# devmentality/LEAStereo

Measured on AMD Instinct MI355X. Metric: stereo pairs/s at 576×960 D=192, 1/2/4/8 GPU; EPE vs reference, higher is better.
Workload: dtype f32; 1 GPU; SceneFlow 576x960 D=192 fp32, batch 1 per GPU (BASELINE configs[1]); height=576, width=960, maxdisp=192, global_batch=1, parallelism=dp1 (pairs sharded over ranks, no collective in the step), launch=hip graph replay

## Files before the change

### include/leastereo_hip.h

```cpp
#ifndef LEASTEREO_HIP_H
#define LEASTEREO_HIP_H

#include <stddef.h>
#include <stdint.h>

#ifdef __cplusplus
extern "C" {
#endif

#define LEA_ABI_VERSION 14

#define LEA_F32 0
#define LEA_BF16 1

#define LEA_OK 0
#define LEA_E_INVALID 1001
#define LEA_E_UNSUPPORTED 1002

#define LEA_RELU 1u
#define LEA_RESIDUAL 2u
#define LEA_PAIR_SUM 4u

int lea_abi_version(void);
const char* lea_last_error(void);
// ... 10 lines not shown
                      const void* x2, int64_t x2_bstride, int cin2,
                      const float* w_packed, const float* scale, const float* shift,
                      const void* residual, int64_t r_bstride,
                      void* y, int64_t y_bstride,
                      int B, int cin, int cout, int D, int H, int W, int k,
                      unsigned flags, int dtype, void* stream);

int lea_conv1x1_heads(const void* x, int64_t x_bstride, const void* x2, int64_t x2_bstride,
                      int cin2, const float* w_packed,
                      const float* scale_a, const float* shift_a, void* y_a, int64_t ya_bstride,
                      int cout_a, unsigned flags_a,
                      const float* scale_b, const float* shift_b, void* y_b, int64_t yb_bstride,
                      int cout_b, unsigned flags_b,
                      int B, int cin, int D, int H, int W, int dtype, void* stream);
const char* lea_conv1x1_heads_kernel_name(int B, int cout, int D, int H, int W);

int lea_conv3d_bnrelu_resampled(const void* x, int64_t x_bstride, int Di, int Hi, int Wi,
                                const float* w_packed, const float* scale, const float* shift,
                                const void* residual, int64_t r_bstride,
                                void* y, int64_t y_bstride,
                                int B, int cin, int cout, int D, int H, int W, int k,
                                unsigned flags, int dtype, void* stream);

int lea_conv3d_bnrelu_costvolume(const void* left, const void* right, int64_t f_bstride,
                                 const float* w_packed, const float* scale, const float* shift,
                                 void* y, int64_t y_bstride, int B, int C, int cout, int D3,
                                 int H, int W, unsigned flags, int dtype, void* stream);
const char* lea_conv3d_costvolume_kernel_name(int B, int cout, int D3, int H, int W);

const char* lea_conv3d_kernel_name(int B, int cout, int D, int H, int W, int k, int resampled);
// ... 291 lines not shown
```

### include/leastereo_hip_tuning.h

```cpp
#ifndef LEASTEREO_HIP_TUNING_H
#define LEASTEREO_HIP_TUNING_H

#ifdef __cplusplus
extern "C" {
#endif

int lea_conv3d_set_tile_override(int nt, int tw, int td);

int lea_conv3d_set_rs_gather(int on);

int lea_conv1x1_set_vector(int on);

int lea_conv3d_bf16_set_tile_override(int th, int td, int mt);

int lea_conv3d_bf16_set_variant(int variant);

int lea_conv3d_bf16_set_stream1x1(int on);

int lea_conv3d_bf16_set_pair_split(int on);

int lea_resample_bf16_set_batch(int k);

int lea_resample_bf16_set_cols(int on);

// ... 25 lines not shown

int lea_conv3d_wino2_set_pipeline(int on);

int lea_conv3d_wino2p_set_wpre(int on);

int lea_conv3d_wino44_set(int on);

int lea_conv3d_wino44_set_upre(int on);

int lea_conv3d_wino44_set_sched(int s);

int lea_conv3d_wino44_set_group(int g);

int lea_conv3d_wino_set_epi_buf(int on);

int lea_conv3d_wino_set_small_cout(int mode);

int lea_conv3d_wino_set_block48(int on);

int lea_rectify_set_tile(int mode);

#ifdef __cplusplus
}
#endif
#endif
```

### leastereo_amd/_lib.py

```python
from __future__ import annotations

import ctypes
import os
import threading

LIB_PATH = os.environ.get(
    "LEASTEREO_HIP_LIB",
    os.path.join(os.path.dirname(os.path.abspath(__file__)), "libleastereo_hip.so"))

ABI_VERSION = 14
LEA_F32 = 0
LEA_BF16 = 1
LEA_RELU = 1
LEA_RESIDUAL = 2
LEA_PAIR_SUM = 4
LEA_CVS_TMAJOR = 8
LEA_E_INVALID = 1001

_p = ctypes.c_void_p
_i = ctypes.c_int
_i64 = ctypes.c_int64
_u = ctypes.c_uint

SIGNATURES = {
    "lea_abi_version": (_i, []),
    "lea_last_error": (ctypes.c_char_p, []),
    "lea_build_cost_volume": (_i, [_p, _p, _p, _i, _i, _i, _i, _i, _i, _p]),
    "lea_conv3d_packed_floats": (ctypes.c_size_t, [_i, _i, _i]),
    "lea_conv3d_pack_weights": (_i, [_p, _p, _i, _i, _i, _p]),
    "lea_conv3d_bnrelu": (_i, [_p, _i64, _p, _i64, _i, _p, _p, _p, _p, _i64, _p, _i64,
                               _i, _i, _i, _i, _i, _i, _i, _u, _i, _p]),
    "lea_conv1x1_heads": (_i, [_p, _i64, _p, _i64, _i, _p, _p, _p, _p, _i64, _i, _u, _p, _p, _p, _i64, _i, _u,
                               _i, _i, _i, _i, _i, _i, _p]),
    "lea_conv1x1_heads_kernel_name": (ctypes.c_char_p, [_i, _i, _i, _i, _i]),
    "lea_conv3d_bnrelu_resampled": (_i, [_p, _i64, _i, _i, _i, _p, _p, _p, _p, _i64, _p, _i64,
                                         _i, _i, _i, _i, _i, _i, _i, _u, _i, _p]),
    "lea_conv3d_kernel_name": (ctypes.c_char_p, [_i, _i, _i, _i, _i, _i, _i]),
    "lea_conv3d_set_tile_override": (_i, [_i, _i, _i]),
    "lea_conv3d_bnrelu_costvolume": (_i, [_p, _p, _i64, _p, _p, _p, _p, _i64, _i, _i, _i, _i, _i,
                                          _i, _u, _i, _p]),
    "lea_conv3d_costvolume_kernel_name": (ctypes.c_char_p, [_i, _i, _i, _i, _i]),
    "lea_conv2d_packed_floats": (ctypes.c_size_t, [_i, _i]),
    "lea_conv2d_pack_weights": (_i, [_p, _p, _i, _i, _p]),
    "lea_conv2d_bnrelu": (_i, [_p, _i64, _p, _p, _p, _p, _i64, _p, _i64, _i, _i, _i, _i, _i, _u,
                               _i, _p]),
    "lea_conv2d_kernel_name": (ctypes.c_char_p, [_i, _i, _i, _i]),
    "lea_conv2d_s3_bnrelu": (_i, [_p, _i64, _p, _p, _p, _p, _i64, _i, _i, _i, _i, _i, _u, _i, _p]),
    "lea_feature_stem_bnrelu": (_i, [_p, _i64, _p, _p, _p, _p, _p, _p, _p, _i64, _i, _i, _i, _i, _i, _i,
                                     _i, _p]),
# ... 83 lines not shown
    "lea_conv3d_wino2_set_halo16": (_i, [_i]),
    "lea_conv3d_wino2_set_lane_halo16": (_i, [_i]),
    "lea_conv3d_wino_set_fence": (_i, [_i]),
    "lea_resample_set_mode": (_i, [_i]),
    "lea_conv2d_set_small": (_i, [_i]),
    "lea_conv2d_kernel_name_cin": (ctypes.c_char_p, [_i, _i, _i, _i, _i]),
    "lea_conv2d_bnrelu_pair": (_i, [_p, _i64, _p, _p, _p, _p, _i64, _p, _i64, _p, _i64, _i, _i, _i, _i, _i,
                                    _i, _u, _p]),
    "lea_conv3d_wino2_set_pipeline": (_i, [_i]),
    "lea_conv3d_wino2p_set_wpre": (_i, [_i]),
    "lea_conv3d_wino44_set": (_i, [_i]),
    "lea_conv3d_wino44_set_upre": (_i, [_i]),
    "lea_conv3d_wino44_set_sched": (_i, [_i]),
    "lea_conv3d_wino44_set_group": (_i, [_i]),
    "lea_conv3d_wino_set_epi_buf": (_i, [_i]),
    "lea_conv3d_set_rs_gather": (_i, [_i]),
    "lea_conv1x1_set_vector": (_i, [_i]),
    "lea_conv3d_bf16_set_stream1x1": (_i, [_i]),
    "lea_conv3d_wino_set_small_cout": (_i, [_i]),
    "lea_conv3d_wino_set_block48": (_i, [_i]),
    "lea_cv_stem_split_weights": (_i, [_p, _p, _p, _i, _i, _p]),
    "lea_cv_stem_combine": (_i, [_p, _i64, _p, _i64, _p, _p, _p, _i64, _i, _i, _i, _i, _i, _u, _i,
                                 _p]),
    "lea_cv_stem_map_windows": (_i, [_i, _i, ctypes.POINTER(_i), ctypes.POINTER(_i)]),
    "lea_conv2d_windowed_tiles": (_i, [_i, _i, _i, _i, _i, ctypes.POINTER(_i)]),
    "lea_conv2d_bnrelu_windowed": (_i, [_p, _i64, _p, _p, _p, _p, _i64, _i, _i, _i, _i, _i, _i, _i, _i, _i, _i,
                                        _u, _i, _p]),
    "lea_cv_stem_down2_supported": (_i, [_i, _i, _i, _i, _i]),
    "lea_cv_stem_combine_down2": (_i, [_p, _i64, _p, _i64, _p, _p, _p, _i64, _p, _i64, _i, _i, _i, _i, _i,
                                       _u, _i, _p]),
# ... 54 lines not shown
            _lib = lib
    return _lib


TUNING_ENV = {"LEASTEREO_WINO2_WALK": "lea_conv3d_wino2_set_walk",
              "LEASTEREO_HALO16": "lea_conv3d_wino2_set_halo16",
              "LEASTEREO_LANE_HALO16": "lea_conv3d_wino2_set_lane_halo16",
              "LEASTEREO_WINO_FENCE": "lea_conv3d_wino_set_fence",
              "LEASTEREO_RESAMPLE_MODE": "lea_resample_set_mode",
              "LEASTEREO_CONV2D_SMALL": "lea_conv2d_set_small",
              "LEASTEREO_WINO2_PIPE": "lea_conv3d_wino2_set_pipeline",
              "LEASTEREO_WINO2P_WPRE": "lea_conv3d_wino2p_set_wpre",
              "LEASTEREO_WINO44": "lea_conv3d_wino44_set",
              "LEASTEREO_WINO44_UPRE": "lea_conv3d_wino44_set_upre",
              "LEASTEREO_EPI_BUF": "lea_conv3d_wino_set_epi_buf",
              "LEASTEREO_RS_GATHER": "lea_conv3d_set_rs_gather",
              "LEASTEREO_1X1_VEC": "lea_conv1x1_set_vector",
              "LEASTEREO_BF16_1X1": "lea_conv3d_bf16_set_stream1x1",
              "LEASTEREO_RESAMPLE_K": "lea_resample_bf16_set_batch",
              "LEASTEREO_RESAMPLE_COLS": "lea_resample_bf16_set_cols",
              "LEASTEREO_W22": "lea_conv3d_wino_set_w22",
              "LEASTEREO_PAIR_SPLIT": "lea_conv3d_bf16_set_pair_split",
              "LEASTEREO_DISP_REG": "lea_disparity_set_register_form",
              "LEASTEREO_TAPSUM_ROWS": "lea_tapsum_set_rows"}


def _apply_env_tuning(lib):
    for var, fn in TUNING_ENV.items():
        if os.environ.get(var):
            if getattr(lib, fn)(int(os.environ[var])) != 0:
# ... 8 lines not shown
```

### leastereo_amd/csrc/conv3d.hip

```cpp
#include "conv3d_impl.h"

namespace lea {

template <int KS, int MT, int NT, int TW, bool RS>
__global__ __launch_bounds__(kConvThreads, 2) void conv3d_reg_kernel(const ConvArgs a) {
  using C = TileCfg<KS, MT, NT, TW>;
  constexpr int CIN_B = C::CIN_B;
  __shared__ __attribute__((aligned(16))) float smem[C::STAGE];
  __shared__ Axis tabs[RS ? (KS + C::RH + C::RW) : 1];
  float* xs = smem;
  float* ws = smem + C::XS;

  const int tid = threadIdx.x;
  const int lane = tid & 63;
  const int wave = tid >> 6;
  const int tile = blockIdx.x;
  const int h0 = (tile / a.tiles_w) * C::TH;
  const int w0 = (tile % a.tiles_w) * TW;
  const int d0 = blockIdx.y;
  const int b = blockIdx.z / a.ncob;
  const int co0 = (blockIdx.z - b * a.ncob) * C::COP;
  const int nchunks = (a.cin + CIN_B - 1) / CIN_B;
  const float* wp = a.wp + (long long)(co0 / C::COP) * nchunks * C::WS;
  const long long HW = (long long)a.H * a.W;
// ... 297 lines not shown
      }
    }
  }
}

template <int MT, int NT, bool VEC>
__global__ __launch_bounds__(kConvThreads) void conv1x1_kernel(const ConvArgs a) {
  conv1x1_body<MT, NT, VEC, false>(a, Conv1x1HeadB{});
}

template <int MT, int NT, bool VEC>
__global__ __launch_bounds__(kConvThreads) void conv1x1_heads_kernel(const ConvArgs a, const Conv1x1HeadB hb) {
  conv1x1_body<MT, NT, VEC, true>(a, hb);
}

template <int COUT>
__global__ __launch_bounds__(kConvThreads) void conv3d_valu_kernel(const ConvArgs a) {
  constexpr int TH = 8, TW = 64, RH = TH + 2, RW = TW + 2, PLANE = RH * RW, IMG = 3 * PLANE;
  constexpr int CIN_B = PackCfg<3, 1>::CIN_B;
  constexpr int CIS = (IMG + 15) / 16 * 16;
  constexpr int STAGE = CIN_B * CIS;
  constexpr int XSLOTS = (IMG + 63) / 64;
  constexpr int XSLOTS_W = (XSLOTS + kConvWaves - 1) / kConvWaves;
  constexpr int CHUNK = PackCfg<3, 1>::CHUNK;
  __shared__ __attribute__((aligned(16))) float smem[2 * STAGE];

  const int tid = threadIdx.x;
  const int lane = tid & 63;
  const int wave = __builtin_amdgcn_readfirstlane(tid >> 6);
  const int h0 = (blockIdx.x / a.tiles_w) * TH;
// ... 564 lines not shown
  a.wp = w_packed;
  a.scale = scale_a;
  a.shift = shift_a;
  a.y = (float*)y_a;
  a.ybs = ya_bstride;
  a.cin = cin;
  a.cout = cout_a + cout_b;
  a.D = D;
  a.H = H;
  a.W = W;
  a.flags = flags_a;
  const Conv1x1HeadB hb{(float*)y_b, yb_bstride, scale_b, shift_b, cout_a, flags_b};
  const Plan p = make_plan(B, a.cout, D, H, W, 1, false);
  a.ncob = (a.cout + p.mt * 16 - 1) / (p.mt * 16);
  return run_1x1(p, a, B, as_stream(stream), &hb);
}

extern "C" size_t lea_conv2d_packed_floats(int cout, int cin) {
  if (cout <= 0 || cin <= 0) return 0;
  return lea::packed_floats_2d(cout, cin);
}

extern "C" int lea_conv2d_pack_weights(const float* w, float* packed, int cout, int cin,
                                       void* stream) {
  using namespace lea;
  clear_error();
  LEA_CHECK_ARG(w && packed, "lea_conv2d_pack_weights: null pointer");
  LEA_CHECK_ARG(cout > 0 && cin > 0, "lea_conv2d_pack_weights: bad shape cout=%d cin=%d", cout, cin);
  const long long total = (long long)packed_floats_2d(cout, cin);
  const int threads = 256;
// ... 252 lines not shown
```

### leastereo_amd/csrc/conv3d_wino.hip

```cpp
#include "wino_common.h"

namespace lea {
namespace wino {

template <int F, int Q, int MT, int NP, int TD, bool H16 = false>
struct Cfg {
  static constexpr bool DP = MT == 0;
  static constexpr int MTE = DP ? 1 : MT;
  static constexpr int TDA = DP ? 1 : TD;
  static constexpr int NSTEP = DP ? 12 : 9;
  static_assert(!DP || TD == 2, "a depth-paired tile covers two output planes");
  static constexpr int NX = F + 2;
  static constexpr int COP = 16 * MTE;
  static constexpr bool SWZ = (COP % 32) == 0;
  static constexpr int RPG = 16 / Q;
  static constexpr int TW = F * Q;
  static constexpr int TH = 4 * NP * RPG;
  static constexpr int RH = TH + 2, RW = TW + 2;
  static constexpr int PLANE = RH * RW;
  static constexpr int PLANES = TD + 2;
  static constexpr int IMG = PLANES * PLANE;
  static constexpr int XSLOTS = (IMG + 63) / 64;
  static constexpr int CIS = conflict_free_cis<F, Q>(64 * XSLOTS, RW);
  static constexpr int RWA = TW + 8;
// ... 53 lines not shown
  const int q8 = nblk / 8, r8 = nblk % 8;
  const int lin = (xcd < r8 ? xcd * (q8 + 1) : r8 * (q8 + 1) + (xcd - r8) * q8) + idx;
  const int spw = a.spw > 0 ? a.spw : 1;
  const int ngz = (a.ndz + spw - 1) / spw;
  const int cob = lin % a.ncob;
  const int rest = lin / a.ncob;
  const int gz = rest % ngz;
  const int tile = (rest / ngz) % a.ntiles;
  const int b = rest / (ngz * a.ntiles);
  const int h0 = (tile / a.tiles_w) * C::TH;
  const int w0 = (tile % a.tiles_w) * C::TW;
  const int dz0 = gz * spw, ngroups = min(spw, a.ndz - dz0);
  const int co0 = cob * C::COP;
  const int nchunks = a.cin / CIN_B;
  const int nitems = ngroups * nchunks;
  const float* wp = a.wp + (long long)cob * nchunks * C::WS;
  const int HW = a.H * a.W;
  const unsigned nrec = (unsigned)(HW * a.D) * 4u;

  unsigned hwo[XSLOTS_W];
  int pln[XSLOTS_W], wco[CV ? XSLOTS_W : 1];
#pragma unroll
  for (int t = 0; t < XSLOTS_W; ++t) {
    const int e = (wave + kConvWaves * t) * 64 + lane;
    unsigned v = 0xFFFFFFF0u;
    int pl = -1000, wc_ = 0;
    if (e < C::IMG) {
      const int p = e / C::PLANE;
      const int r = e - p * C::PLANE;
      const int rr = r / C::RW;
// ... 44 lines not shown
      if constexpr (CV) {
        const bool okc = ok && wco[t] >= d;
        voff[t] = okc ? hwo[t] : 0xFFFFFFF0u;
        voffr[t] = okc ? hwo[t] - (unsigned)d * 4u : 0xFFFFFFF0u;
      } else {
        voff[t] = ok ? hwo[t] + (unsigned)d * (unsigned)HW * 4u : 0xFFFFFFF0u;
      }
    }
  };

  auto issue = [&](int item, float* st) {
    const int ch = item % nchunks;
    if (ch == 0) set_group((dz0 + item / nchunks) * TD);
    const float* wsrc = wp + (long long)ch * C::WS;
    float* wdst = st + C::XS;
#pragma unroll
    for (int t = 0; t < WSLOTS_W; ++t) {
      const int j = wave + kConvWaves * t;
      if (j < WSLOTS)
        dma_dwordx4(wsrc + j * 256 + lane * 4, lds0 + 4 * (unsigned)(wdst - smem + j * 256));
    }
    const long long cvol = CV ? (long long)HW : (long long)HW * a.D;
    const unsigned crec = CV ? (unsigned)HW * 4u : nrec;
    if constexpr (H16) {
#pragma unroll
      for (int t = 0; t < T16; ++t) {
        const int k = wave + kConvWaves * t, ci = k / P16;
        const int c = ch * CIN_B + ci;
        const float* base = c < a.cin1 ? a.x + (long long)b * a.xbs + (long long)c * cvol
                                       : a.x2 + (long long)b * a.x2bs + (long long)(c - a.cin1) * cvol;
        const __amdgpu_buffer_rsrc_t rs = __builtin_amdgcn_make_buffer_rsrc((void*)base, 0, crec, 0x00020000);
        const int cb = C::cbh(0) + ci * C::CSH;
        if (ok16[t]) dma_dwordx4_buf(rs, voff16[t], lds0 + 4 * (unsigned)(st - smem + cb + (k % P16) * 256));
      }
      return;
// ... 468 lines not shown
}

struct Plan {
  int f, q, mt, np, td;
  bool d2;
  Plan2 p2;
  bool h16;
};

int g_override[3] = {0, 0, 0};
int g_variant = 0;
int g_spw = 0;
int g_small16 = 0;
int g_block48 = 1;
int g_epibuf = 1;
int g_halo16 = 1;
int g_pipe = 1;
int g_wpre = 1;
int g_fence = 1;
int g_lane16 = 2;
int g_w22 = 0;
inline int host_mt(int cout) {
  if (g_small16 && cout <= 8) return 1;
  const int mt = mt_of(cout);
  return (mt == 3 && !g_block48) ? 2 : mt;
}
inline long long staged_floats(int cout, int cin) {
  const int mt = host_mt(cout), cop = cop_of(mt), nstep = mt == 0 ? 12 : 9;
  return (long long)((cout + cop - 1) / cop) * (cin / CIN_B) * nstep * 3 * CIN_B * cop + 256;
}
// ... 111 lines not shown
    conv3d_wino_kernel<F, Q, MT, NP, TD, CV><<<dim3((unsigned)n_), kConvThreads, 0, st>>>(a); \
    return launch_status("lea_conv3d(wino)");                                                \
  }
#define LEA_WINO_TILES(CV)                                                                                  \
  LEA_WINO_CASE(2, 16, 1, 1, 1, CV) LEA_WINO_CASE(2, 16, 1, 1, 2, CV) LEA_WINO_CASE(2, 16, 1, 2, 1, CV)     \
  LEA_WINO_CASE(2, 16, 1, 2, 2, CV) LEA_WINO_CASE(2, 16, 2, 1, 1, CV) LEA_WINO_CASE(2, 16, 2, 1, 2, CV)     \
  LEA_WINO_CASE(2, 16, 2, 2, 1, CV) LEA_WINO_CASE(2, 16, 2, 2, 2, CV) LEA_WINO_CASE(2, 16, 3, 1, 1, CV)     \
  LEA_WINO_CASE(2, 16, 3, 1, 2, CV) LEA_WINO_CASE(4, 16, 1, 1, 1, CV) LEA_WINO_CASE(4, 16, 1, 1, 2, CV)     \
  LEA_WINO_CASE(4, 16, 2, 1, 1, CV) LEA_WINO_CASE(4, 16, 2, 1, 2, CV) LEA_WINO_CASE(4, 8, 1, 1, 1, CV)      \
  LEA_WINO_CASE(4, 8, 1, 1, 2, CV) LEA_WINO_CASE(4, 8, 2, 1, 1, CV) LEA_WINO_CASE(4, 8, 2, 1, 2, CV)      \
  LEA_WINO_CASE(4, 8, 3, 1, 1, CV) LEA_WINO_CASE(4, 16, 0, 1, 2, CV) LEA_WINO_CASE(4, 8, 0, 1, 2, CV)

int run(const Plan& p, ConvArgs a, int B, hipStream_t st, bool cv) {
  if (p.d2) return run2(p.p2, a, B, st, cv);
  a.ncob = (a.cout + cop_of(p.mt) - 1) / cop_of(p.mt);
  if (p.h16) {
    using C_ = Cfg<4, 16, 0, 1, 2, true>;
    a.tiles_w = (a.W + C_::TW - 1) / C_::TW;
    a.ntiles = a.tiles_w * ((a.H + C_::TH - 1) / C_::TH);
    a.ndz = (a.D + 1) / 2;
    a.spw = std::max(1, std::min(g_spw > 0 ? g_spw : auto_walk(a, B, 2), a.ndz));
    const long long n_ = (long long)a.ntiles * ((a.ndz + a.spw - 1) / a.spw) * B * a.ncob;
    LEA_CHECK_ARG(n_ < (1LL << 31), "lea_conv3d(wino): grid too large");
    a.nblk = (int)n_;
    if (g_fence)
      conv3d_wino_kernel<4, 16, 0, 1, 2, false, true, true><<<dim3((unsigned)n_), kConvThreads, 0, st>>>(a);
    else
      conv3d_wino_kernel<4, 16, 0, 1, 2, false, true><<<dim3((unsigned)n_), kConvThreads, 0, st>>>(a);
    return launch_status("lea_conv3d(wino)");
  }
// ... 129 lines not shown
  wino::g_override[2] = f;
  return 0;
}

extern "C" int lea_conv3d_wino_set_block48(int on) {
  clear_error();
  LEA_CHECK_ARG(on == 0 || on == 1, "lea_conv3d_wino_set_block48: on=%d", on);
  wino::g_block48 = on;
  return 0;
}

extern "C" int lea_conv3d_wino_set_epi_buf(int on) {
  clear_error();
  LEA_CHECK_ARG(on == 0 || on == 1, "lea_conv3d_wino_set_epi_buf: on=%d", on);
  wino::g_epibuf = on;
  return 0;
}

extern "C" int lea_conv3d_wino_set_small_cout(int mode) {
  clear_error();
  LEA_CHECK_ARG(mode == 0 || mode == 1, "lea_conv3d_wino_set_small_cout: mode=%d", mode);
  wino::g_small16 = mode;
  return 0;
}

extern "C" int lea_conv3d_wino2_set_pipeline(int on) {
  clear_error();
  LEA_CHECK_ARG(on == 0 || on == 1, "lea_conv3d_wino2_set_pipeline: on=%d", on);
  wino::g_pipe = on;
  return 0;
// ... 144 lines not shown
  if (B <= 0 || cin <= 0 || cout <= 0 || cout > 8 || D < 2 || H < 2 || W < 4 || D % 2 || H % 2 || W % 4 ||
      cin % CIN_B)
    return 0;
  if ((long long)D * H * W * 4 >= (1LL << 32) || (long long)(cout + 47) * D * H * W >= (1LL << 31)) return 0;
  if (!g_epibuf || g_w22 == 2 || g_variant != 0 || g_override[0] != 0) return 0;
  Plan p = make_plan(B, cout, D, H, W);
  if (p.mt != 0 || p.d2 || p.f != 4 || p.np != 1 || p.td != 2) return 0;
  plan_halo16(p, false, W, a, cin);
  if (a && !epi_buf_ok(*a)) return 0;
  if (p.q == 16) return (p.h16 && g_fence) ? 16 : 0;
  return p.q == 8 ? 8 : 0;
}

static int run_dp_down2(ConvArgs a, int B, int q, bool only, hipStream_t st) {
  a.ncob = 1;
  const int tw = 4 * q, th = 4 * (16 / q);
  a.tiles_w = (a.W + tw - 1) / tw;
  a.ntiles = a.tiles_w * ((a.H + th - 1) / th);
  a.ndz = (a.D + 1) / 2;
  a.spw = std::max(1, std::min(g_spw > 0 ? g_spw : auto_walk(a, B, 2), a.ndz));
  const long long n_ = (long long)a.ntiles * ((a.ndz + a.spw - 1) / a.spw) * B * a.ncob;
  LEA_CHECK_ARG(n_ < (1LL << 31), "lea_conv3d_bnrelu_wino_dp_down2: grid too large");
  a.nblk = (int)n_;
  const dim3 grid((unsigned)n_);
  if (q == 16) {
    if (only)
      conv3d_wino_dp_down2_kernel<16, true><<<grid, kConvThreads, 0, st>>>(a);
    else
      conv3d_wino_dp_down2_kernel<16, false><<<grid, kConvThreads, 0, st>>>(a);
  } else {
// ... 202 lines not shown
```

### leastereo_amd/csrc/wino_common.h

```cpp
#pragma once
#include "conv3d_impl.h"

namespace lea {
namespace wino {

constexpr int CIN_B = 4;

__host__ __device__ constexpr int mt_of(int cout) {
  return cout <= 8 ? 0 : cout <= 16 ? 1 : (cout % 32 != 0 && cout % 48 == 0) ? 3 : 2;
}
__host__ __device__ constexpr int cop_of(int mt) { return 16 * (mt > 0 ? mt : 1); }

template <int F, int Q>
__host__ __device__ constexpr int lane_dword(int lane, int cis, int rw) {
  return (lane >> 4) * cis + ((lane & 15) / Q) * rw + F * ((lane & 15) % Q);
}
template <int F, int Q>
__host__ __device__ constexpr int conflict_free_cis(int img, int rw) {
  for (int cis = img + (img & 1);; cis += 2) {
    bool used[64] = {};
    bool ok = true;
    for (int l = 0; l < 32 && ok; ++l)
      for (int k = 0; k < 2 && ok; ++k) {
        const int bank = (lane_dword<F, Q>(l, cis, rw) + k) % 64;
// ... 14 lines not shown
}
__device__ __forceinline__ void dma_dwordx4_buf(__amdgpu_buffer_rsrc_t rs, unsigned voff, unsigned lds) {
  unsigned keep;
  asm volatile("s_mov_b32 %0, m0\n\ts_mov_b32 m0, %3\n\ts_nop 0\n\tbuffer_load_dwordx4 %1, %2, 0 offen lds\n\ts_mov_b32 m0, %0"
               : "=&s"(keep) : "v"(voff), "s"(rs), "s"(lds) : "memory");
}
__device__ __forceinline__ void dma_dwordx4(const float* src, unsigned lds) {
  unsigned keep;
  asm volatile("s_mov_b32 %0, m0\n\ts_mov_b32 m0, %2\n\ts_nop 0\n\tglobal_load_lds_dwordx4 %1, off\n\ts_mov_b32 m0, %0"
               : "=&s"(keep) : "v"(src), "s"(lds) : "memory");
}

__device__ __forceinline__ int a_col(int m, int ci, int n, bool swz) { return ((swz ? (m ^ (ci & 1)) : m) * 16) + n; }

constexpr unsigned kEpiBuf = 1u << 16;
constexpr unsigned kPairSum = LEA_PAIR_SUM;
constexpr unsigned kEpiOob = 0xFFFFFF00u;
typedef unsigned u32x4_t __attribute__((ext_vector_type(4)));
typedef unsigned u32x2_t __attribute__((ext_vector_type(2)));
typedef float f32x2 __attribute__((ext_vector_type(2)));
__device__ __forceinline__ __amdgpu_buffer_rsrc_t block_rsrc(const float* base, long long bytes) {
  return __builtin_amdgcn_make_buffer_rsrc((void*)base, 0, (int)(unsigned)bytes, 0x00020000);
}
__device__ __forceinline__ f32x4 buf_load4(__amdgpu_buffer_rsrc_t rs, unsigned off) {
  return __builtin_bit_cast(f32x4, __builtin_amdgcn_raw_buffer_load_b128(rs, off, 0, 0));
}
__device__ __forceinline__ void buf_store4(__amdgpu_buffer_rsrc_t rs, unsigned off, f32x4 v) {
  __builtin_amdgcn_raw_buffer_store_b128(__builtin_bit_cast(u32x4_t, v), rs, off, 0, 0);
}
template <int NST>
// ... 59 lines not shown
```

### leastereo_amd/executor.py

```python
from __future__ import annotations

import os
from dataclasses import dataclass

import torch

from . import kernels
from .arch import scale_dimension


def _stacked(fl: torch.Tensor, fr: torch.Tensor) -> torch.Tensor:
    if (fl.is_contiguous() and fr.is_contiguous() and fl.shape == fr.shape and fl.dtype == fr.dtype
            and fl.device == fr.device
            and fl.untyped_storage().data_ptr() == fr.untyped_storage().data_ptr()
            and fr.data_ptr() == fl.data_ptr() + fl.numel() * fl.element_size()):
        return fl.as_strided((2 * fl.shape[0],) + tuple(fl.shape[1:]), fl.stride())
    return torch.cat((fl, fr), 0)


@dataclass
class ConvParams:
    packed: torch.Tensor
    scale: torch.Tensor | None
    shift: torch.Tensor | None
# ... 385 lines not shown
                    dst.add_(t)
                else:
                    dst.copy_(t)
                written.add(step)
            states.append(dst)
        return prev_input, out


class MatchingExecutor(CellGraphExecutor):
    SPLIT_S1_GROUP48 = os.environ.get("LEASTEREO_SPLIT_GROUP48", "1") != "0"
    PAIR_STEPS = WINOGRAD and os.environ.get("LEASTEREO_PAIR_STEPS", "0") != "0"
    FUSED_DOWN = os.environ.get("LEASTEREO_FUSED_DOWN", "1") != "0"
    FUSED_DOWN_CELLS = os.environ.get("LEASTEREO_FUSED_DOWN_CELLS", "1") != "0"
    WINDOWED_MAPS = os.environ.get("LEASTEREO_WINDOWED_MAPS", "1") != "0"
    FANOUT_1X1 = os.environ.get("LEASTEREO_FANOUT_1X1", "1") != "0"

    def run(self, x):
        return self._from_stem0(self.conv("stem0", x))

    def run_features(self, fl, fr, maxdisp):
        p = self.p["stem0"]
        if fl.shape[1] * 2 != p.cin:
            raise ValueError(f"stem0 expects {p.cin} cost-volume channels, got 2*{fl.shape[1]}")
        d3 = int(maxdisp / 3)
        if self.cv is not None and kernels.cv_stem_supported(p.cout, d3, fl.shape[3], False):
            return self._from_stem0(*self._cv_stem(fl.unsqueeze(2), fr.unsqueeze(2), d3))
        if p.wino is not None and kernels.wino_preferred(fl.shape[0], p.cout, p.cin, int(maxdisp / 3),
                                                         *fl.shape[2:4]):
            stem0 = kernels.conv3d_bnrelu_costvolume_wino(fl, fr, maxdisp, p.wino, p.cout, p.scale,
                                                          p.shift, p.relu)
# ... 105 lines not shown
                    prev = (outs[4][0], fused)
            elif i == 9 and n == 12:
                fused = self.conv("conv2", outs[4][1], x2=outs[8][1])
                self._emit("conv2", fused)
                prev = (outs[8][0], fused)
            o = self.cell(i, prev[0], prev[1], down=down)
            cell_down, self._cell_down = self._cell_down, None
            self._emit(f"cell{i}", o[1])
            outs.append(o)
            prev = o
        last = outs[-1][1]
        lh = self._volume(last)[1]
        full, half, quarter = (d, h, w), (d // 2, h // 2, w // 2), (d // 4, h // 4, w // 4)
        if lh == h:
            return self._last3_same_size(last)
        if lh == h // 2:
            y = self.conv("last_6", last)
        elif lh == h // 4:
            y = self.conv("last_6", self.conv("last_12", last), size=half)
        elif lh == h // 8:
            y = self.conv("last_12", self.conv("last_24", last), size=quarter)
            y = self.conv("last_6", y, size=half)
        else:
            raise ValueError(f"matching-net output size {tuple(last.shape[2:])} has no head")
        p3 = self.p["last_3"]
        q = self.conv("last_3.taps", y)
        return self._tapsum(q, p3, full)

    @staticmethod
    def _tapsum(q, p3, full):
        return kernels.tapsum_upsample(q, p3.cout, full, p3.scale, p3.shift, p3.relu)

    def _last3_same_size(self, last):
        return self.conv("last_3", last)

    def __init__(self, matching):
        super().__init__(matching)
        with torch.no_grad():
            last3 = matching.last_3.conv.weight
            co, ci = last3.shape[:2]
            taps = last3.permute(0, 2, 3, 4, 1).reshape(co * 27, ci, 1, 1, 1)
            self.p["last_3.taps"] = ConvParams(kernels.pack_conv_weight(taps), None, None,
# ... 3 lines not shown
                wl, wr = kernels.cv_stem_split_weights(matching.stem0.conv.weight)
                self.cv = self._cv_stem_pack(wl, wr)
                if self.WINDOWED_MAPS and not isinstance(self, _C8Layout):
                    co = wl.shape[0] // 9
                    wlt = wl.view(3, 3, co, *wl.shape[1:]).transpose(0, 1).reshape(wl.shape)
                    self.cv_win = (kernels.pack_conv2d_weight_windowed(wlt, 3 * co),
                                   kernels.pack_conv2d_weight_windowed(wr, 3 * co))
        self._use_winograd()


class MatchingExecutorDirect(MatchingExecutor):

    SPLIT_S1_GROUP48 = False
    PAIR_STEPS = False
    FANOUT_1X1 = False

    def __init__(self, matching):
        super().__init__(matching)
        self.cv = self.cv_win = None

    def _use_winograd(self):
        """Direct engine only."""


class FeatureExecutor(CellGraphExecutor):
    FUSED_STEM = os.environ.get("LEASTEREO_FEATURE_STEM", "1") != "0"
    PAIR_S0 = os.environ.get("LEASTEREO_PAIR_S0", "1") != "0"

    def _stems(self, x, c8=False, x2=None):
        p0, p1 = self.p["stem0"], self.p["stem1"]
# ... 89 lines not shown
                                                      p.relu, out)
            x = self._downsampled(x, size)
        if p.kind == "bf16_2d":
            if x2 is not None:
                raise ValueError(f"{name}: 2D conv takes one input")
            return kernels.conv2d_bnrelu_bf16(x, p.packed, p.cout, p.scale, p.shift, p.relu, out,
                                              accumulate, residual)
        return kernels.conv3d_bnrelu_bf16(x, p.packed, p.cout, p.k, p.scale, p.shift, p.relu, out,
                                          accumulate, x2, residual)


class MatchingExecutorBF16(_C8Layout, MatchingExecutor):

    SPLIT_S1_GROUP48 = False
    FANOUT_1X1 = False
    PAIR_STEPS = os.environ.get("LEASTEREO_PAIR_STEPS", "1") != "0"

    def __init__(self, matching):
        from .model import ConvBR
        super().__init__(matching)
        with torch.no_grad():
            for name, p in list(self.p.items()):
                if name == "last_3":
                    continue
                if name == "last_3.taps":
                    w = matching.last_3.conv.weight
                    co, ci = w.shape[:2]
                    taps = w.permute(0, 2, 3, 4, 1).reshape(co * 27, ci, 1, 1, 1)
                    pad = (-taps.shape[0]) % 8
                    taps = torch.cat([taps, taps.new_zeros((pad,) + tuple(taps.shape[1:]))], 0)
# ... 144 lines not shown
```

### leastereo_amd/kernels.py

```python
from __future__ import annotations

import collections
import contextlib
import ctypes
import math
import os

import numpy as np
import torch

from . import _lib
from ._lib import LEA_BF16, LEA_CVS_TMAJOR, LEA_F32, LEA_PAIR_SUM, LEA_RELU, LEA_RESIDUAL, check


def _stream():
    return torch.cuda.current_stream().cuda_stream


ProbeRecord = collections.namedtuple("ProbeRecord", "name flops bytes start end mfma_flops shape")


class KernelProbe:

    def __init__(self, names=None):
# ... 289 lines not shown
        raise ValueError("conv1x1_heads: neither head accumulates or takes a residual")
    _require_cuda(x, x2, packed, scale_a, shift_a, scale_b, shift_b, out_a, out_b)
    b, cin, d, h, w = x.shape
    xbs = _check_volume_view(x, "x")
    x2ptr, x2bs, cin2 = _second_source(x2, b, (d, h, w))
    out_a, abs_ = _out_view(out_a, _act_shape(b, cout_a, (d, h, w)), x.device, name="out_a")
    out_b, bbs = _out_view(out_b, _act_shape(b, cout_b, (d, h, w)), x.device, name="out_b")
    cout = cout_a + cout_b
    _launch("lea_conv1x1_heads", x.data_ptr(), xbs, x2ptr, x2bs, cin2, packed.data_ptr(),
            _ptr(scale_a), _ptr(shift_a), out_a.data_ptr(), abs_, cout_a, _flags(relu_a),
            _ptr(scale_b), _ptr(shift_b), out_b.data_ptr(), bbs, cout_b, _flags(relu_b),
            b, cin + cin2, d, h, w, LEA_F32,
            probe=lambda: _conv_record(b, cin + cin2, cout, d, h, w, 1, False, b * d * h * w, False,
                                       name=_decode(_lib.load().lea_conv1x1_heads_kernel_name(b, cout, d, h, w))))
    return out_a, out_b


def costvolume_kernel_name(b, cout, d3, h, w):
    return _decode(_lib.load().lea_conv3d_costvolume_kernel_name(b, cout, d3, h, w))


def conv3d_bnrelu_costvolume(fl: torch.Tensor, fr: torch.Tensor, maxdisp: int, packed: torch.Tensor,
                             cout: int, scale: torch.Tensor | None, shift: torch.Tensor | None,
                             relu: bool = True) -> torch.Tensor:
    _require_cuda(fl, fr, packed, scale, shift)
    b, c, h, w = _feature_pair(fl, fr)
    d3 = int(maxdisp / 3)
    out = torch.empty((b, cout, d3, h, w), device=fl.device, dtype=fl.dtype)
    _launch("lea_conv3d_bnrelu_costvolume", fl.data_ptr(), fr.data_ptr(), fl.stride(0), packed.data_ptr(),
            _ptr(scale), _ptr(shift), out.data_ptr(), out.stride(0), b, c, cout, d3, h, w, _flags(relu), LEA_F32,
# ... 1337 lines not shown
```

Before: 166.3 pairs/s.

## Fuse head 1x1 conv chain into one kernel and keep Winograd weights resident

```diff
diff --git a/include/leastereo_hip.h b/include/leastereo_hip.h
--- a/include/leastereo_hip.h
+++ b/include/leastereo_hip.h
@@ -48,6 +48,13 @@
                       int cout_b, unsigned flags_b,
                       int B, int cin, int D, int H, int W, int dtype, void* stream);
 const char* lea_conv1x1_heads_kernel_name(int B, int cout, int D, int H, int W);
+
+int lea_conv1x1_chain(const void* x, int64_t x_bstride,
+                      const float* w1_packed, const float* scale1, const float* shift1, unsigned flags1,
+                      const float* w2_packed, const float* scale2, const float* shift2, unsigned flags2,
+                      void* y, int64_t y_bstride,
+                      int B, int c0, int c1, int c2, int D, int H, int W, int dtype, void* stream);
+const char* lea_conv1x1_chain_kernel_name(int B, int c1, int c2, int D, int H, int W);
 
 int lea_conv3d_bnrelu_resampled(const void* x, int64_t x_bstride, int Di, int Hi, int Wi,
                                 const float* w_packed, const float* scale, const float* shift,
diff --git a/include/leastereo_hip_tuning.h b/include/leastereo_hip_tuning.h
--- a/include/leastereo_hip_tuning.h
+++ b/include/leastereo_hip_tuning.h
@@ -63,6 +63,8 @@
 
 int lea_conv3d_wino_set_epi_buf(int on);
 
+int lea_conv3d_wino_set_wresident(int on);
+
 int lea_conv3d_wino_set_small_cout(int mode);
 
 int lea_conv3d_wino_set_block48(int on);
diff --git a/leastereo_amd/_lib.py b/leastereo_amd/_lib.py
--- a/leastereo_amd/_lib.py
+++ b/leastereo_amd/_lib.py
@@ -16,6 +16,7 @@
 LEA_PAIR_SUM = 4
 LEA_CVS_TMAJOR = 8
 LEA_E_INVALID = 1001
+LEA_E_UNSUPPORTED = 1002
 
 _p = ctypes.c_void_p
 _i = ctypes.c_int
@@ -33,6 +34,9 @@
     "lea_conv1x1_heads": (_i, [_p, _i64, _p, _i64, _i, _p, _p, _p, _p, _i64, _i, _u, _p, _p, _p, _i64, _i, _u,
                                _i, _i, _i, _i, _i, _i, _p]),
     "lea_conv1x1_heads_kernel_name": (ctypes.c_char_p, [_i, _i, _i, _i, _i]),
+    "lea_conv1x1_chain": (_i, [_p, _i64, _p, _p, _p, _u, _p, _p, _p, _u, _p, _i64, _i, _i, _i, _i, _i, _i, _i,
+                               _i, _p]),
+    "lea_conv1x1_chain_kernel_name": (ctypes.c_char_p, [_i, _i, _i, _i, _i, _i]),
     "lea_conv3d_bnrelu_resampled": (_i, [_p, _i64, _i, _i, _i, _p, _p, _p, _p, _i64, _p, _i64,
                                          _i, _i, _i, _i, _i, _i, _i, _u, _i, _p]),
     "lea_conv3d_kernel_name": (ctypes.c_char_p, [_i, _i, _i, _i, _i, _i, _i]),
@@ -146,6 +150,7 @@
     "lea_conv3d_wino44_set_sched": (_i, [_i]),
     "lea_conv3d_wino44_set_group": (_i, [_i]),
     "lea_conv3d_wino_set_epi_buf": (_i, [_i]),
+    "lea_conv3d_wino_set_wresident": (_i, [_i]),
     "lea_conv3d_set_rs_gather": (_i, [_i]),
     "lea_conv1x1_set_vector": (_i, [_i]),
     "lea_conv3d_bf16_set_stream1x1": (_i, [_i]),
@@ -230,6 +235,7 @@
               "LEASTEREO_WINO44": "lea_conv3d_wino44_set",
               "LEASTEREO_WINO44_UPRE": "lea_conv3d_wino44_set_upre",
               "LEASTEREO_EPI_BUF": "lea_conv3d_wino_set_epi_buf",
+              "LEASTEREO_WINO_WRES": "lea_conv3d_wino_set_wresident",
               "LEASTEREO_RS_GATHER": "lea_conv3d_set_rs_gather",
               "LEASTEREO_1X1_VEC": "lea_conv1x1_set_vector",
               "LEASTEREO_BF16_1X1": "lea_conv3d_bf16_set_stream1x1",
diff --git a/leastereo_amd/csrc/conv3d.hip b/leastereo_amd/csrc/conv3d.hip
--- a/leastereo_amd/csrc/conv3d.hip
+++ b/leastereo_amd/csrc/conv3d.hip
@@ -335,6 +335,173 @@
   conv1x1_body<MT, NT, VEC, true>(a, hb);
 }
 
+struct Conv1x1Second {
+  const float* wp;
+  const float* scale;
+  const float* shift;
+  int cout;
+  unsigned flags;
+};
+
+constexpr int kChainTile = 32 * 16 + 8 * 16;
+
+__device__ __forceinline__ void wave_lds_sync() {
+  __builtin_amdgcn_fence(__ATOMIC_RELEASE, "wavefront");
+  __builtin_amdgcn_wave_barrier();
+  __builtin_amdgcn_fence(__ATOMIC_ACQUIRE, "wavefront");
+}
+
+template <int MT1, int MT2, int NT, bool VEC>
+__global__ __launch_bounds__(kConvThreads, 5) void conv1x1_chain_kernel(const ConvArgs a, const Conv1x1Second sb) {
+  using P = PackCfg<1, MT1>;
+  using P2 = PackCfg<1, MT2>;
+  static_assert(MT1 <= 2 && MT2 <= 2, "the middle tensor is one cout block and one K chunk");
+  constexpr int CIN_B = P::CIN_B;
+  constexpr int KS = CIN_B / 4;
+  using vecf = float __attribute__((ext_vector_type(NT)));
+  __shared__ __attribute__((aligned(16))) float ws[P::CHUNK];
+  __shared__ __attribute__((aligned(16))) float ws2[P2::CHUNK];
+  __shared__ float tiles[kConvWaves][kChainTile];
+  __shared__ float ep1[2][32];
+  const int tid = threadIdx.x;
+  const int lane = tid & 63;
+  const int wave = tid >> 6;
+  const int b = blockIdx.y;
+  const int nchunks = (a.cin + CIN_B - 1) / CIN_B;
+  const long long V = (long long)a.D * a.H * a.W;
+  const long long v0 = ((long long)blockIdx.x * kConvWaves + wave) * NT * 16;
+  const int kq = lane >> 4, n = lane & 15;
+  auto vox = [&](int j) -> long long { return VEC ? v0 + NT * n + j : v0 + j * 16 + n; };
+  const bool full = VEC && vox(NT - 1) < V;
+
+  {
+    const float4* src = reinterpret_cast<const float4*>(sb.wp);
+    float4* dst = reinterpret_cast<float4*>(ws2);
+#pragma unroll
+    for (int i = tid; i < P2::CHUNK / 4; i += kConvThreads) dst[i] = src[i];
+    if (tid < 32) {
+      ep1[0][tid] = (a.scale && tid < a.cout) ? a.scale[tid] : 1.f;
+      ep1[1][tid] = (a.shift && tid < a.cout) ? a.shift[tid] : 0.f;
+    }
+  }
+
+  constexpr int MTX = MT1 > MT2 ? MT1 : MT2;
+  f32x4 acc[MTX][NT];
+#pragma unroll
+  for (int m = 0; m < MT1; ++m)
+#pragma unroll
+    for (int j = 0; j < NT; ++j) acc[m][j] = f32x4{0.f, 0.f, 0.f, 0.f};
+
+  for (int ch = 0; ch < nchunks; ++ch) {
+    float bv[KS][NT];
+#pragma unroll
+    for (int s = 0; s < KS; ++s) {
+      const int c = ch * CIN_B + 4 * s + kq;
+      const float* src = a.x + (long long)b * a.xbs + (long long)c * V;
+      if (VEC && full && c < a.cin) {
+        const vecf t = *reinterpret_cast<const vecf*>(src + vox(0));
+#pragma unroll
+        for (int j = 0; j < NT; ++j) bv[s][j] = t[j];
+      } else {
+#pragma unroll
+        for (int j = 0; j < NT; ++j) {
+          const long long v = vox(j);
+          bv[s][j] = (c < a.cin && v < V) ? src[v] : 0.f;
+        }
+      }
+    }
+    __syncthreads();
+    {
+      const float4* src = reinterpret_cast<const float4*>(a.wp + (long long)ch * P::CHUNK);
+      float4* dst = reinterpret_cast<float4*>(ws);
+#pragma unroll
+      for (int i = tid; i < P::CHUNK / 4; i += kConvThreads) dst[i] = src[i];
+    }
+    __syncthreads();
+#pragma unroll
+    for (int s = 0; s < KS; ++s) {
+      float av[MT1];
+#pragma unroll
+      for (int m = 0; m < MT1; ++m) av[m] = ws[(4 * s + kq) * P::COPS + a_col<1, MT1>(m, kq, n)];
+#pragma unroll
+      for (int m = 0; m < MT1; ++m)
+#pragma unroll
+        for (int j = 0; j < NT; ++j)
+          acc[m][j] = __builtin_amdgcn_mfma_f32_16x16x4f32(av[m], bv[s][j], acc[m][j], 0, 0, 0);
+    }
+  }
+
+  int lane2 = lane;
+  asm volatile("" : "+v"(lane2));
+  const int kq2 = lane2 >> 4, n2 = lane2 & 15;
+  auto vox2 = [&](int j) -> long long { return VEC ? v0 + NT * n2 + j : v0 + j * 16 + n2; };
+  const bool full2 = VEC && vox2(NT - 1) < V;
+
+  const bool relu1 = a.flags & LEA_RELU;
+  float* tile = tiles[wave];
+
+#pragma unroll
+  for (int j = 0; j < NT; ++j) {
+    __builtin_amdgcn_sched_barrier(0);
+#pragma unroll
+    for (int m = 0; m < MT1; ++m)
+#pragma unroll
+      for (int r = 0; r < 4; ++r) {
+        const int c = m * 16 + kq2 * 4 + r;
+        float val = acc[m][j][r] * ep1[0][c] + ep1[1][c];
+        if (relu1) val = fmaxf(val, 0.f);
+        tile[c * 16 + (c >> 2) * 16 + n2] = c < a.cout ? val : 0.f;
+      }
+    wave_lds_sync();
+    float bv2[KS];
+#pragma unroll
+    for (int s = 0; s < KS; ++s) bv2[s] = 4 * s < 16 * MT1 ? tile[(4 * s + kq2) * 16 + s * 16 + n2] : 0.f;
+    wave_lds_sync();
+#pragma unroll
+    for (int m = 0; m < MT2; ++m) acc[m][j] = f32x4{0.f, 0.f, 0.f, 0.f};
+#pragma unroll
+    for (int s = 0; s < KS; ++s) {
+      float av[MT2];
+#pragma unroll
+      for (int m = 0; m < MT2; ++m) av[m] = ws2[(4 * s + kq2) * P2::COPS + a_col<1, MT2>(m, kq2, n2)];
+#pragma unroll
+      for (int m = 0; m < MT2; ++m)
+        acc[m][j] = __builtin_amdgcn_mfma_f32_16x16x4f32(av[m], bv2[s], acc[m][j], 0, 0, 0);
+    }
+  }
+
+  const bool relu2 = sb.flags & LEA_RELU;
+  float* y = a.y + (long long)b * a.ybs;
+#pragma unroll
+  for (int m = 0; m < MT2; ++m) {
+#pragma unroll
+    for (int r = 0; r < 4; ++r) {
+      const int co = m * 16 + kq2 * 4 + r;
+      if (co >= sb.cout) continue;
+      const float sc = sb.scale ? sb.scale[co] : 1.f;
+      const float sh = sb.shift ? sb.shift[co] : 0.f;
+      if (VEC && full2) {
+        vecf val;
+#pragma unroll
+        for (int j = 0; j < NT; ++j) {
+          val[j] = acc[m][j][r] * sc + sh;
+          if (relu2) val[j] = fmaxf(val[j], 0.f);
+        }
+        *reinterpret_cast<vecf*>(y + (long long)co * V + vox2(0)) = val;
+        continue;
+      }
+#pragma unroll
+      for (int j = 0; j < NT; ++j) {
+        const long long v = vox2(j);
+        if (v >= V) continue;
+        float val = acc[m][j][r] * sc + sh;
+        if (relu2) val = fmaxf(val, 0.f);
+        y[(long long)co * V + v] = val;
+      }
+    }
+  }
+}
+
 template <int COUT>
 __global__ __launch_bounds__(kConvThreads) void conv3d_valu_kernel(const ConvArgs a) {
   constexpr int TH = 8, TW = 64, RH = TH + 2, RW = TW + 2, PLANE = RH * RW, IMG = 3 * PLANE;
@@ -929,6 +1096,85 @@
   const Plan p = make_plan(B, a.cout, D, H, W, 1, false);
   a.ncob = (a.cout + p.mt * 16 - 1) / (p.mt * 16);
   return run_1x1(p, a, B, as_stream(stream), &hb);
+}
+
+namespace lea {
+
+template <int MT1, int MT2, int NT>
+int launch_chain(const ConvArgs& a, const Conv1x1Second& sb, int B, hipStream_t st) {
+  const long long vox = (long long)a.D * a.H * a.W;
+  const long long per = kConvWaves * NT * 16;
+  const long long gx = (vox + per - 1) / per;
+  LEA_CHECK_ARG(gx < (1LL << 31) && B <= 65535, "lea_conv1x1_chain: grid too large");
+  auto al = [](const void* q) { return ((uintptr_t)q % (NT * 4)) == 0; };
+  const bool vec = g_1x1_vec && vox % NT == 0 && al(a.x) && al(a.y) && a.xbs % NT == 0 && a.ybs % NT == 0;
+  const dim3 grid((unsigned)gx, B);
+  if (vec) conv1x1_chain_kernel<MT1, MT2, NT, true><<<grid, kConvThreads, 0, st>>>(a, sb);
+  else conv1x1_chain_kernel<MT1, MT2, NT, false><<<grid, kConvThreads, 0, st>>>(a, sb);
+  return launch_status("lea_conv1x1_chain");
+}
+
+template <int MT1, int MT2>
+int run_chain(int nt, const ConvArgs& a, const Conv1x1Second& sb, int B, hipStream_t st) {
+  return nt == 4 ? launch_chain<MT1, MT2, 4>(a, sb, B, st) : launch_chain<MT1, MT2, 2>(a, sb, B, st);
+}
+
+}
+
+extern "C" const char* lea_conv1x1_chain_kernel_name(int B, int c1, int c2, int D, int H, int W) {
+  if (B <= 0 || c1 <= 0 || c1 > 32 || c2 <= 0 || c2 > 32 || D <= 0 || H <= 0 || W <= 0) return nullptr;
+  const lea::Plan p = lea::make_plan(B, c2, D, H, W, 1, false);
+  snprintf(lea::g_name, sizeof(lea::g_name), "conv1x1_chain_kernel<%d, %d, %d>", lea::mt_for(c1), p.mt, p.nt);
+  return lea::g_name;
+}
+
+extern "C" int lea_conv1x1_chain(const void* x, int64_t x_bstride, const float* w1_packed, const float* scale1,
+                                 const float* shift1, unsigned flags1, const float* w2_packed,
+                                 const float* scale2, const float* shift2, unsigned flags2, void* y,
+                                 int64_t y_bstride, int B, int c0, int c1, int c2, int D, int H, int W,
+                                 int dtype, void* stream) {
+  using namespace lea;
+  clear_error();
+  LEA_CHECK_FLAGS(flags1, LEA_RELU, "lea_conv1x1_chain");
+  LEA_CHECK_FLAGS(flags2, LEA_RELU, "lea_conv1x1_chain");
+  LEA_CHECK_ARG(x && w1_packed && w2_packed && y, "lea_conv1x1_chain: null pointer");
+  LEA_CHECK_ARG((scale1 == nullptr) == (shift1 == nullptr) && (scale2 == nullptr) == (shift2 == nullptr),
+                "lea_conv1x1_chain: a conv's scale/shift must both be set or both NULL");
+  LEA_CHECK_ARG(B > 0 && c0 > 0 && c1 > 0 && c2 > 0 && D > 0 && H > 0 && W > 0,
+                "lea_conv1x1_chain: bad shape B=%d channels %d -> %d -> %d D=%d H=%d W=%d", B, c0, c1, c2, D, H, W);
+  const long long vox = (long long)D * H * W;
+  LEA_CHECK_ARG(vox * 4 < (1LL << 32) && (long long)(c2 + 63) * vox < (1LL << 31),
+                "lea_conv1x1_chain: volume too large");
+  LEA_CHECK_ARG(x != y, "lea_conv1x1_chain: input aliases the output");
+  if (dtype != LEA_F32) {
+    set_error("lea_conv1x1_chain: dtype %d unsupported", dtype);
+    return LEA_E_UNSUPPORTED;
+  }
+  if (c1 > 32 || c2 > 32) {
+    set_error("lea_conv1x1_chain: %d -> %d -> %d: the middle and the output take at most 32 channels", c0, c1, c2);
+    return LEA_E_UNSUPPORTED;
+  }
+  ConvArgs a{};
+  a.x = (const float*)x;
+  a.xbs = x_bstride;
+  a.cin1 = c0;
+  a.wp = w1_packed;
+  a.scale = scale1;
+  a.shift = shift1;
+  a.y = (float*)y;
+  a.ybs = y_bstride;
+  a.cin = c0;
+  a.cout = c1;
+  a.D = D;
+  a.H = H;
+  a.W = W;
+  a.flags = flags1;
+  a.ncob = 1;
+  const Conv1x1Second sb{w2_packed, scale2, shift2, c2, flags2};
+  const int nt = make_plan(B, c2, D, H, W, 1, false).nt;
+  hipStream_t st = as_stream(stream);
+  if (c1 <= 16) return c2 <= 16 ? run_chain<1, 1>(nt, a, sb, B, st) : run_chain<1, 2>(nt, a, sb, B, st);
+  return c2 <= 16 ? run_chain<2, 1>(nt, a, sb, B, st) : run_chain<2, 2>(nt, a, sb, B, st);
 }
 
 extern "C" size_t lea_conv2d_packed_floats(int cout, int cin) {
diff --git a/leastereo_amd/csrc/conv3d_wino.hip b/leastereo_amd/csrc/conv3d_wino.hip
--- a/leastereo_amd/csrc/conv3d_wino.hip
+++ b/leastereo_amd/csrc/conv3d_wino.hip
@@ -91,6 +91,7 @@
   const int co0 = cob * C::COP;
   const int nchunks = a.cin / CIN_B;
   const int nitems = ngroups * nchunks;
+  const bool wres = (a.flags & kWRes) && nchunks <= 2;
   const float* wp = a.wp + (long long)cob * nchunks * C::WS;
   const int HW = a.H * a.W;
   const unsigned nrec = (unsigned)(HW * a.D) * 4u;
@@ -165,11 +166,13 @@
     if (ch == 0) set_group((dz0 + item / nchunks) * TD);
     const float* wsrc = wp + (long long)ch * C::WS;
     float* wdst = st + C::XS;
-#pragma unroll
-    for (int t = 0; t < WSLOTS_W; ++t) {
-      const int j = wave + kConvWaves * t;
-      if (j < WSLOTS)
-        dma_dwordx4(wsrc + j * 256 + lane * 4, lds0 + 4 * (unsigned)(wdst - smem + j * 256));
+    if (!(wres && item >= 2)) {
+#pragma unroll
+      for (int t = 0; t < WSLOTS_W; ++t) {
+        const int j = wave + kConvWaves * t;
+        if (j < WSLOTS)
+          dma_dwordx4(wsrc + j * 256 + lane * 4, lds0 + 4 * (unsigned)(wdst - smem + j * 256));
+      }
     }
     const long long cvol = CV ? (long long)HW : (long long)HW * a.D;
     const unsigned crec = CV ? (unsigned)HW * 4u : nrec;
@@ -668,6 +671,7 @@
 int g_small16 = 0;
 int g_block48 = 1;
 int g_epibuf = 1;
+int g_wres = 1;
 int g_halo16 = 1;
 int g_pipe = 1;
 int g_wpre = 1;
@@ -809,6 +813,7 @@
 int run(const Plan& p, ConvArgs a, int B, hipStream_t st, bool cv) {
   if (p.d2) return run2(p.p2, a, B, st, cv);
   a.ncob = (a.cout + cop_of(p.mt) - 1) / cop_of(p.mt);
+  if (g_wres) a.flags |= kWRes;
   if (p.h16) {
     using C_ = Cfg<4, 16, 0, 1, 2, true>;
     a.tiles_w = (a.W + C_::TW - 1) / C_::TW;
@@ -968,6 +973,13 @@
   clear_error();
   LEA_CHECK_ARG(on == 0 || on == 1, "lea_conv3d_wino_set_epi_buf: on=%d", on);
   wino::g_epibuf = on;
+  return 0;
+}
+
+extern "C" int lea_conv3d_wino_set_wresident(int on) {
+  clear_error();
+  LEA_CHECK_ARG(on == 0 || on == 1, "lea_conv3d_wino_set_wresident: on=%d", on);
+  wino::g_wres = on;
   return 0;
 }
 
@@ -1142,6 +1154,7 @@
 
 static int run_dp_down2(ConvArgs a, int B, int q, bool only, hipStream_t st) {
   a.ncob = 1;
+  if (g_wres) a.flags |= kWRes;
   const int tw = 4 * q, th = 4 * (16 / q);
   a.tiles_w = (a.W + tw - 1) / tw;
   a.ntiles = a.tiles_w * ((a.H + th - 1) / th);
diff --git a/leastereo_amd/csrc/wino_common.h b/leastereo_amd/csrc/wino_common.h
--- a/leastereo_amd/csrc/wino_common.h
+++ b/leastereo_amd/csrc/wino_common.h
@@ -52,6 +52,7 @@
 __device__ __forceinline__ int a_col(int m, int ci, int n, bool swz) { return ((swz ? (m ^ (ci & 1)) : m) * 16) + n; }
 
 constexpr unsigned kEpiBuf = 1u << 16;
+constexpr unsigned kWRes = 1u << 17;
 constexpr unsigned kPairSum = LEA_PAIR_SUM;
 constexpr unsigned kEpiOob = 0xFFFFFF00u;
 typedef unsigned u32x4_t __attribute__((ext_vector_type(4)));
diff --git a/leastereo_amd/executor.py b/leastereo_amd/executor.py
--- a/leastereo_amd/executor.py
+++ b/leastereo_amd/executor.py
@@ -423,6 +423,7 @@
     FUSED_DOWN_CELLS = os.environ.get("LEASTEREO_FUSED_DOWN_CELLS", "1") != "0"
     WINDOWED_MAPS = os.environ.get("LEASTEREO_WINDOWED_MAPS", "1") != "0"
     FANOUT_1X1 = os.environ.get("LEASTEREO_FANOUT_1X1", "1") != "0"
+    HEAD_CHAIN = os.environ.get("LEASTEREO_HEAD_CHAIN", "1") != "0"
 
     def run(self, x):
         return self._from_stem0(self.conv("stem0", x))
@@ -558,6 +559,11 @@
         full, half, quarter = (d, h, w), (d // 2, h // 2, w // 2), (d // 4, h // 4, w // 4)
         if lh == h:
             return self._last3_same_size(last)
+        if lh == h // 2 and self._head_chain_takes(last):
+            p6, pt = self.p["last_6"], self.p["last_3.taps"]
+            q = kernels.conv1x1_chain(last, p6.packed, p6.cout, p6.scale, p6.shift, p6.relu,
+                                      pt.packed, pt.cout, pt.scale, pt.shift, pt.relu)
+            return self._tapsum(q, self.p["last_3"], full)
         if lh == h // 2:
             y = self.conv("last_6", last)
         elif lh == h // 4:
@@ -570,6 +576,14 @@
         p3 = self.p["last_3"]
         q = self.conv("last_3.taps", y)
         return self._tapsum(q, p3, full)
+
+    def _head_chain_takes(self, last):
+        p6, pt = self.p["last_6"], self.p["last_3.taps"]
+        return (self.HEAD_CHAIN and last.is_cuda and last.dtype == torch.float32 and last.dim() == 5
+                and p6.kind == "3d" and pt.kind == "3d" and p6.k == 1 and pt.k == 1
+                and last.shape[1] == p6.cin and p6.cout == pt.cin
+                and kernels.conv1x1_chain_kernel_name(last.shape[0], p6.cout, pt.cout,
+                                                      *last.shape[2:5]) is not None)
 
     @staticmethod
     def _tapsum(q, p3, full):
@@ -603,6 +617,7 @@
     SPLIT_S1_GROUP48 = False
     PAIR_STEPS = False
     FANOUT_1X1 = False
+    HEAD_CHAIN = False
 
     def __init__(self, matching):
         super().__init__(matching)
@@ -722,6 +737,7 @@
 
     SPLIT_S1_GROUP48 = False
     FANOUT_1X1 = False
+    HEAD_CHAIN = False
     PAIR_STEPS = os.environ.get("LEASTEREO_PAIR_STEPS", "1") != "0"
 
     def __init__(self, matching):
diff --git a/leastereo_amd/kernels.py b/leastereo_amd/kernels.py
--- a/leastereo_amd/kernels.py
+++ b/leastereo_amd/kernels.py
@@ -327,6 +327,27 @@
             probe=lambda: _conv_record(b, cin + cin2, cout, d, h, w, 1, False, b * d * h * w, False,
                                        name=_decode(_lib.load().lea_conv1x1_heads_kernel_name(b, cout, d, h, w))))
     return out_a, out_b
+
+
+def conv1x1_chain_kernel_name(b, c1, c2, d, h, w):
+    return _decode(_lib.load().lea_conv1x1_chain_kernel_name(b, c1, c2, d, h, w))
+
+
+def conv1x1_chain(x: torch.Tensor, packed1: torch.Tensor, c1: int, scale1, shift1, relu1: bool,
+                  packed2: torch.Tensor, c2: int, scale2, shift2, relu2: bool,
+                  out: torch.Tensor | None = None) -> torch.Tensor:
+    _require_cuda(x, packed1, packed2, scale1, shift1, scale2, shift2, out)
+    b, c0, d, h, w = x.shape
+    xbs = _check_volume_view(x, "x")
+    out, ybs = _out_view(out, _act_shape(b, c2, (d, h, w)), x.device, name="out")
+    vox = b * d * h * w
+    _launch("lea_conv1x1_chain", x.data_ptr(), xbs, packed1.data_ptr(), _ptr(scale1), _ptr(shift1), _flags(relu1),
+            packed2.data_ptr(), _ptr(scale2), _ptr(shift2), _flags(relu2), out.data_ptr(), ybs,
+            b, c0, c1, c2, d, h, w, LEA_F32,
+            probe=lambda: _op_record(conv1x1_chain_kernel_name(b, c1, c2, d, h, w), 2.0 * vox * (c0 * c1 + c1 * c2),
+                                     4.0 * vox * (c0 + c2) + 4.0 * (c0 * c1 + c1 * c2),
+                                     shape=(b, c0, c2, d, h, w, 1)))
+    return out
 
 
 def costvolume_kernel_name(b, cout, d3, h, w):
```

Result: no change. 166.9 pairs/s, median of 6 (+0.4%).
